# hyx1999/SAM-Decoding

Measured on AMD Instinct MI355X. Metric: tokens/sec (+ mean accepted tokens), Vicuna-7B bs=1, samd_sam_only draft+verify, higher is better.
Workload: dtype f16

## Files before the change

include/samd_hip.h:

```cpp
#ifndef SAMD_HIP_H
#define SAMD_HIP_H

#include <stdint.h>

#ifdef __cplusplus
extern "C" {
#endif

#define SAMD_OK 0
#define SAMD_E_INVALID (-1)
#define SAMD_E_CAPACITY (-2)
#define SAMD_E_HIP (-3)
#define SAMD_E_IO (-4)
#define SAMD_E_NODEVICE (-5)

#define SAMD_MAX_DRAFT 128
#define SAMD_TOPK 8

#define SAMD_REP_DMETA 0
#define SAMD_REP_VERDICT 16
#define SAMD_REP_TOKENS 24
#define SAMD_REP_KVINDEX 152
#define SAMD_REP_COUNTERS 280
#define SAMD_REP_META 288
// ... 77 lines not shown
    uint64_t mask_hi[SAMD_MAX_DRAFT];
    int32_t retrieve[SAMD_MAX_DRAFT * SAMD_MAX_DRAFT];
} samd_draft_host_t;

typedef struct samd_verdict_host {
    int32_t best, accept, next_node, next_token;
    int32_t tokens[SAMD_MAX_DRAFT];
    int32_t kv_index[SAMD_MAX_DRAFT];
} samd_verdict_host_t;

int samd_session_create(int32_t max_tokens, samd_session_t **out);
void samd_session_free(samd_session_t *s);
int samd_session_reset(samd_session_t *s, void *stream);

int samd_dyn_add_tokens(samd_session_t *s, const int32_t *d_tokens, int32_t n, const int32_t *d_n, void *stream);
int samd_dyn_walk(samd_session_t *s, const int32_t *d_tokens, int32_t n, int32_t commit, int32_t *d_out, void *stream);
int samd_session_static_walk(samd_session_t *s, const samd_static_t *sam, const int32_t *d_tokens, int32_t n,
                             const int32_t *d_n, int32_t commit, int32_t *d_out, void *stream);
int samd_session_export(samd_session_t *s, int64_t out_info[10], int32_t *h_link, int32_t *h_length, int32_t *h_minend,
                        int32_t *h_deg, int32_t *h_edge_tok, int32_t *h_edge_dst, int32_t *h_text, void *stream);
int samd_session_set_cursors(samd_session_t *s, int32_t dyn_index, int32_t dyn_length, int32_t st_index,
                             int32_t st_length, void *stream);

int samd_session_set_start_token(samd_session_t *s, const int32_t *d_src, void *stream);

int samd_session_draft(samd_session_t *s, const samd_static_t *sam, const samd_params_t *p,
                       const int32_t *d_start_token, void *stream);
int samd_session_draft_seq(samd_session_t *s, const samd_params_t *p, int32_t index, int32_t match, int32_t start_token,
                           void *stream);
int samd_session_draft_tree(samd_session_t *s, const samd_static_t *sam, const samd_params_t *p, int32_t index,
                            int32_t match, int32_t start_token, void *stream);
int samd_session_draft_fixed(samd_session_t *s, const samd_static_t *sam, const samd_params_t *p, int32_t source,
                             int32_t index, int32_t start_token, void *stream);
int samd_session_set_draft(samd_session_t *s, const int32_t *d_tokens, const int32_t *d_parent, int32_t n, int32_t type,
                           void *stream);
int samd_session_read_draft(samd_session_t *s, samd_draft_host_t *out, void *stream);
int samd_session_set_draft_if_deferred(samd_session_t *s, const int32_t *d_tokens, const int32_t *d_parent, int32_t n,
                                       int32_t reverse_leaves, void *stream);
int samd_tree_attention_signal(const void *d_q, const void *d_k_cache, const void *d_v_cache, void *d_out, int32_t dtype, int32_t n_q_pad,
                               int32_t n_heads, int32_t n_kv_heads, int32_t head_dim, int64_t max_len, const uint64_t *d_mask,
                               const int32_t *d_cache_length, const int32_t *d_n, float scale, void *d_workspace, int64_t workspace_bytes,
                               int32_t *d_arrive, void *stream);
int samd_gemm_cs_residual_early(const void *d_A, const void *d_Wg, int32_t N, int32_t K, void *d_x, float *d_ssq, int32_t dtype, const int32_t *d_counter,
                                int32_t *d_epoch, int32_t arrivals, void *stream);

int samd_session_report_target(samd_session_t *s, int32_t **out_host);
int samd_report_wait(const int32_t *h_report, int32_t last_seq, int64_t timeout_us);

int samd_session_report_async(samd_session_t *s, int32_t *h_dst, void *stream);

int samd_session_device_views(samd_session_t *s, void *out[16]);

int samd_tree_buffers(const int32_t *d_parent, int32_t n, int32_t reverse_leaves, int32_t *d_position, uint64_t *d_mask,
                      uint8_t *d_mask_bool, int32_t *d_retrieve, int32_t *d_shape, void *stream);


int samd_argmax_rows(const void *d_logits, int32_t dtype, int32_t rows, int64_t vocab, int64_t row_stride,
                     const int32_t *d_rows, int32_t *d_out, void *stream);

int samd_session_accept(samd_session_t *s, const int32_t *d_node_argmax, void *stream);
int samd_session_candidates(samd_session_t *s, int64_t *d_candidates, int32_t *d_rowmap, int32_t capacity, void *stream);
int samd_session_step_given(samd_session_t *s, const samd_static_t *sam, const samd_params_t *p, const int32_t *d_best_accept,
                            const int32_t *d_next_token, void *stream);
int samd_session_read_verdict(samd_session_t *s, samd_verdict_host_t *out, void *stream);
int samd_session_commit(samd_session_t *s, const samd_static_t *sam, void *stream);
int samd_session_step(samd_session_t *s, const samd_static_t *sam, const samd_params_t *p,
// ... 188 lines not shown
```

sam-decoding_amd/csrc/sam_device.h:

```cpp
#pragma once
#include <hip/hip_runtime.h>
#include "samd_common.h"

#define WAVE 64
#define PATH_PAD 255

__device__ __forceinline__ int lane_id() { return threadIdx.x & (WAVE - 1); }

__device__ __forceinline__ void wave_mem_sync() { __builtin_amdgcn_fence(__ATOMIC_SEQ_CST, "workgroup"); }

__device__ __forceinline__ int spill_search(const SamEdge *tab, int deg, int tok) {
    const uint32_t m = samd_spill_slots(deg);
    uint32_t h = samd_spill_hash(tok, m);
    for (uint32_t probes = 0; probes < m; probes++) {
        const SamEdge e = tab[h];
        if (e.tok == tok) return e.dst;
        if (e.tok == -1) return -1;
        h = (h + 1) & (m - 1);
    }
    return -1;
}

__device__ __forceinline__ int st_transfer(const StaticDev &S, int &idx, int &len, int tok) {
    int visited = 0;
// ... 561 lines not shown
    double h_prob[8 * SAMD_MAX_DRAFT + 8];
    int h_tok[8 * SAMD_MAX_DRAFT + 8], h_idx[8 * SAMD_MAX_DRAFT + 8], h_anc[8 * SAMD_MAX_DRAFT + 8], h_dep[8 * SAMD_MAX_DRAFT + 8];
    int dep_cnt[SAMD_MAX_DRAFT + 2];
    int c_tok[SAMD_TOPK], c_dst[SAMD_TOPK], c_cnt[SAMD_TOPK];
    int pop_ok, pop_tok, pop_idx, pop_anc, pop_dep; double pop_prob;
};

__device__ __forceinline__ void path_fill(StepShared &sh, int rows) {
    const uint4 pad = make_uint4(0xFFFFFFFFu, 0xFFFFFFFFu, 0xFFFFFFFFu, 0xFFFFFFFFu);
    static_assert(PATH_PAD == 255 && SAMD_MAX_DRAFT % 16 == 0, "");
    uint4 *p = reinterpret_cast<uint4 *>(&sh.path[0][0]);
    for (int k = lane_id(); k < rows * (SAMD_MAX_DRAFT / 16); k += WAVE) p[k] = pad;
}

__device__ __forceinline__ int seq_draft_var(StepShared &sh, const int *text, int n_text, int endpos, int n, int start) {
    const int lo = endpos + 1;
    int hi = endpos + n; hi = hi > n_text ? n_text : hi;
    const int m = 1 + (hi > lo ? hi - lo : 0);
    for (int i = lane_id(); i < m; i += WAVE) { sh.tokens[i] = (i == 0) ? start : text[endpos + i]; sh.parent[i] = i - 1; }
    __syncthreads();
    return m;
}

__device__ __forceinline__ int seq_draft_fixed(StepShared &sh, const int *text, int n_text, int endpos, int n_predicts, int start) {
    for (int i = lane_id(); i < n_predicts; i += WAVE) {
        int v = 0;
        if (i == 0) v = start; else if (endpos + i < n_text) v = text[endpos + i];
        sh.tokens[i] = v; sh.parent[i] = i - 1;
    }
    __syncthreads();
    return n_predicts;
}

__device__ __forceinline__ void hq_set(StepShared &sh, int pos, double p, int t, int i, int a, int d) {
    sh.h_prob[pos] = p; sh.h_tok[pos] = t; sh.h_idx[pos] = i; sh.h_anc[pos] = a; sh.h_dep[pos] = d;
}
__device__ __forceinline__ void hq_move(StepShared &sh, int dst, int src) {
    sh.h_prob[dst] = sh.h_prob[src]; sh.h_tok[dst] = sh.h_tok[src]; sh.h_idx[dst] = sh.h_idx[src];
    sh.h_anc[dst] = sh.h_anc[src]; sh.h_dep[dst] = sh.h_dep[src];
}
__device__ __forceinline__ void hq_siftdown(StepShared &sh, int start, int pos, double p, int t, int i, int a, int d) {
    while (pos > start) {
        const int par = (pos - 1) >> 1;
        if (p < sh.h_prob[par]) { hq_move(sh, pos, par); pos = par; continue; }
        break;
    }
    hq_set(sh, pos, p, t, i, a, d);
}
__device__ __forceinline__ void hq_push(StepShared &sh, int &hn, double p, int t, int i, int a, int d) {
    hn++;
    hq_siftdown(sh, 0, hn - 1, p, t, i, a, d);
}
__device__ __forceinline__ void hq_pop(StepShared &sh, int &hn, double &p, int &t, int &i, int &a, int &d) {
    hn--;
    const double lp = sh.h_prob[hn]; const int lt = sh.h_tok[hn], li = sh.h_idx[hn], la = sh.h_anc[hn], ld = sh.h_dep[hn];
    if (hn == 0) { p = lp; t = lt; i = li; a = la; d = ld; return; }
    p = sh.h_prob[0]; t = sh.h_tok[0]; i = sh.h_idx[0]; a = sh.h_anc[0]; d = sh.h_dep[0];
    int pos = 0, child = 1;
    while (child < hn) {
        const int right = child + 1;
        if (right < hn && !(sh.h_prob[child] < sh.h_prob[right])) child = right;
        hq_move(sh, pos, child); pos = child; child = 2 * pos + 1;
    }
    hq_siftdown(sh, 0, pos, lp, lt, li, la, ld);
}

__device__ __forceinline__ int tree_draft(StepShared &sh, const StaticDev &S, int index, int n, int K, int start) {
    const int lane = lane_id();
    int hn = 0, m = 0;
    for (int k = lane; k < SAMD_MAX_DRAFT + 2; k += WAVE) sh.dep_cnt[k] = 0;
    __syncthreads();
    if (lane == 0) hq_push(sh, hn, -1.0, start, index, -1, 0);
    __syncthreads();
    while (m != n) {
        if (lane == 0) {
            int ok = 0; double p = 0; int t = 0, i = 0, a = 0, d = 0;
            while (hn > 0) {
                hq_pop(sh, hn, p, t, i, a, d);
                if (sh.dep_cnt[d] + 1 > K) continue;
                sh.dep_cnt[d] += 1; ok = 1; break;
            }
            sh.pop_ok = ok; sh.pop_prob = p; sh.pop_tok = t; sh.pop_idx = i; sh.pop_anc = a; sh.pop_dep = d;
        }
        __syncthreads();
        if (!sh.pop_ok) break;
        const int cur = m;
        if (lane == 0) { sh.tokens[m] = sh.pop_tok; sh.parent[m] = sh.pop_anc; }
        m++;
        if (m == n) break;
        const int4 *np = reinterpret_cast<const int4 *>(S.nodes + sh.pop_idx);
        const int4 w1 = np[1];
        const int le = lane < SAMD_INLINE_EDGES ? lane : 0;
        const int2 ie = *reinterpret_cast<const int2 *>(reinterpret_cast<const int *>(np) + SAMD_EDGE_WORD(le));
        const int sp = reinterpret_cast<const int *>(np)[14];
        const int cnt_pre = S.topk_cnt ? S.topk_cnt[(size_t)sh.pop_idx * SAMD_TOPK + (lane & (SAMD_TOPK - 1))] : 0;
        int kk = w1.y < SAMD_TOPK ? w1.y : SAMD_TOPK; kk = kk < K ? kk : K;
        if (lane < kk) {
            int tk = ie.x, ds = ie.y;
            if (lane >= SAMD_INLINE_EDGES) { const SamEdge ed = S.spill[sp + lane - SAMD_INLINE_EDGES]; tk = ed.tok; ds = ed.dst; }
            sh.c_tok[lane] = tk; sh.c_dst[lane] = ds; sh.c_cnt[lane] = S.topk_cnt ? cnt_pre : S.nodes[ds].aux;
        }
        __syncthreads();
        if (lane == 0) {
            const double cnt_sum = (double)w1.x, pp = sh.pop_prob;
            const int dep = sh.pop_dep + 1;
            for (int j = 0; j < kk; j++) {
                const double n_prob = (double)sh.c_cnt[j] / cnt_sum;
                hq_push(sh, hn, pp * n_prob, sh.c_tok[j], sh.c_dst[j], cur, dep);
            }
        }
        __syncthreads();
    }
    __syncthreads();
    return m;
}

__device__ __forceinline__ void build_buffers(StepShared &sh, int n, int reverse, int &n_leaves, int &max_depth) {
    const int lane = lane_id();
    if (lane == 0) { sh.child_mask[0] = 0ull; sh.child_mask[1] = 0ull; }
    __syncthreads();
    for (int i = lane; i < n; i += WAVE) {
        const int p = sh.parent[i];
        if (i == 0) sh.parent[0] = -1;
        else if (p < 0 || p >= i) sh.parent[i] = 0;
    }
    __syncthreads();
    int md = 0;
    for (int i = lane; i < n; i += WAVE) {
        int depth = 0; unsigned long long m = 0ull, mh = 0ull;
        for (int j = i; j != -1; j = sh.parent[j]) { if (j < 64) m |= 1ull << j; else mh |= 1ull << (j - 64); depth++; }
        depth -= 1;
        sh.position[i] = depth; sh.mask[i] = m; sh.mask_hi[i] = mh;
        if (i > 0) { const int p = sh.parent[i]; atomicOr(&sh.child_mask[p >> 6], 1ull << (p & 63)); }
        md = depth + 1 > md ? depth + 1 : md;
    }
    for (int o = 32; o > 0; o >>= 1) { int v = __shfl_xor(md, o); md = v > md ? v : md; }
    __syncthreads();
    const int n0 = n < 64 ? n : 64, n1 = n > 64 ? n - 64 : 0;
    const unsigned long long valid0 = n0 >= 64 ? ~0ull : ((1ull << n0) - 1ull), valid1 = n1 >= 64 ? ~0ull : ((1ull << n1) - 1ull);
    const unsigned long long leaf0 = valid0 & ~sh.child_mask[0], leaf1 = valid1 & ~sh.child_mask[1];
    const int nl0 = __popcll(leaf0), nl = nl0 + __popcll(leaf1);
    path_fill(sh, nl);
    __syncthreads();
    for (int i = lane; i < n; i += WAVE) {
        const bool is_leaf = i < 64 ? ((leaf0 >> i) & 1ull) : ((leaf1 >> (i - 64)) & 1ull);
        if (!is_leaf) continue;
        int r = i < 64 ? __popcll(leaf0 & ((1ull << i) - 1ull)) : nl0 + __popcll(leaf1 & ((1ull << (i - 64)) - 1ull));
        if (reverse) r = nl - 1 - r;
        for (int j = i; j != -1; j = sh.parent[j]) sh.path[r][sh.position[j]] = (unsigned char)j;
    }
    __syncthreads();
    n_leaves = nl; max_depth = md;
}

__device__ __forceinline__ void store_draft(const SessionDev &D, StepShared &sh, int type, int n, int n_leaves, int max_depth,
                                            int idx_dyn, int m_dyn, int idx_st, int m_st, int reverse) {
    const int i = lane_id();
    for (int k = i; k < SAMD_MAX_DRAFT; k += WAVE) {
        if (k < n) { D.tokens[k] = sh.tokens[k]; D.parent[k] = sh.parent[k]; D.position[k] = sh.position[k]; D.mask[k] = sh.mask[k]; D.mask_hi[k] = sh.mask_hi[k]; }
        else { D.tokens[k] = 0; D.parent[k] = k - 1; D.position[k] = 0; D.mask[k] = 0ull; D.mask_hi[k] = 0ull; }
    }
    for (int k = i; k < n_leaves * max_depth; k += WAVE) {
        const unsigned char v = sh.path[k / max_depth][k % max_depth];
        D.retrieve[k] = v == PATH_PAD ? -1 : (int)v;
    }
    if (i == 0) {
        D.dmeta[D_TYPE] = type; D.dmeta[D_N] = n; D.dmeta[D_NLEAVES] = n_leaves; D.dmeta[D_MAXDEPTH] = max_depth;
        D.dmeta[D_IDX_DYN] = idx_dyn; D.dmeta[D_MATCH_DYN] = m_dyn; D.dmeta[D_IDX_ST] = idx_st; D.dmeta[D_MATCH_ST] = m_st;
        D.dmeta[8] = reverse;
    }
}

__device__ __forceinline__ void do_draft(const SessionDev &D, const StaticDev &S, bool have_static, const samd_params_t &P,
                                         StepShared &sh, int start) {
    int id = D.meta[M_CUR_IDX], md = D.meta[M_CUR_LEN];
    dyn_transfer(D, id, md, start);
    int is = 0, ms = 0;
    if (have_static) { is = D.meta[M_ST_IDX]; ms = D.meta[M_ST_LEN]; st_transfer(S, is, ms, start); }
    ms -= P.len_bias;
    int type, n;
    if (P.variant == 0) {
        if (md >= ms || !have_static) {
            type = 0;
            n = seq_draft_var(sh, D.text, D.meta[M_NTEXT], D.minend[id], draft_size(md, P.alpha, P.max_predicts), start);
        } else {
            type = 1;
            n = tree_draft(sh, S, is, draft_size(ms, P.alpha, P.max_predicts), P.K, start);
        }
    } else {
        const int best = md > ms ? md : ms;
        if (best >= P.len_threshold) {
            type = 0;
            if (md >= ms || !have_static) {
                int a = id;
                if (a != 0) {
                    const int maxlen = D.meta[M_MAXLEN];
                    int to_end = maxlen - D.minend[a];
                    while (D.link[a] != 0 && P.n_predicts > to_end) { a = D.link[a]; to_end = maxlen - D.minend[a]; }
                }
                n = seq_draft_fixed(sh, D.text, D.meta[M_NTEXT], D.minend[a], P.n_predicts, start);
            } else {
                n = seq_draft_fixed(sh, S.text, S.n_text, S.nodes[is].aux, P.n_predicts, start);
            }
        } else {
            type = 2; n = 1;
            if (lane_id() == 0) { sh.tokens[0] = start; sh.parent[0] = -1; }
            __syncthreads();
        }
    }
    int nl, mxd;
    build_buffers(sh, n, 0, nl, mxd);
    store_draft(D, sh, type, n, nl, mxd, id, md, is, ms, 0);
}

__device__ __forceinline__ void do_accept(const SessionDev &D, StepShared &sh, const int *node_argmax, int type, int n,
                                          int n_leaves, int max_depth, int &accept_out, int &next_token_out) {
    const int i = lane_id();
    for (int k = i; k < n; k += WAVE) sh.node_argmax[k] = node_argmax[k];
    __syncthreads();
    int key = -1;
    for (int row = i; row < n_leaves; row += WAVE) {
        int acc = 0;
        for (int j = 1; j < max_depth; j++) {
            const int cj = sh.path[row][j], pj = sh.path[row][j - 1];
            const int cand = cj == PATH_PAD ? 0 : sh.tokens[cj];
            const int am = sh.node_argmax[pj == PATH_PAD ? n - 1 : pj];
            if (cand != am) break;
            acc++;
        }
        const int kk = acc * SAMD_MAX_DRAFT + (SAMD_MAX_DRAFT - 1 - row);
        key = kk > key ? kk : key;
    }
    for (int o = 32; o > 0; o >>= 1) { int v = __shfl_xor(key, o); key = v > key ? v : key; }
    const int best_acc = key / SAMD_MAX_DRAFT, best = SAMD_MAX_DRAFT - 1 - (key % SAMD_MAX_DRAFT);
    const int a = best_acc + 1;
    for (int k = i; k < a; k += WAVE) {
        const int node = sh.path[best][k];
        const int tk = node == PATH_PAD ? 0 : sh.tokens[node];
        sh.accepted[k] = tk;
        D.acc_tokens[k] = tk;
        D.kv_index[k] = node == PATH_PAD ? -1 : node;
    }
    const int nn_raw = sh.path[best][best_acc];
    const int nn = nn_raw == PATH_PAD ? n - 1 : nn_raw;
    const int next_token = sh.node_argmax[nn];
// ... 42 lines not shown
```

sam-decoding_amd/csrc/sam_kernels.hip:

```cpp
#include <hip/hip_runtime.h>
#include <cstdio>
#include <cstdlib>
#include <cstring>
#include <ctime>
#include <functional>
#include <vector>
#include <hipcub/hipcub.hpp>
#include "sam_device.h"

#define HIPCHK(x) do { hipError_t e_ = (x); if (e_ != hipSuccess) { samd_set_error("%s: %s", #x, hipGetErrorString(e_)); return SAMD_E_HIP; } } while (0)
#define LAUNCHCHK() do { hipError_t e_ = hipGetLastError(); if (e_ != hipSuccess) { samd_set_error("kernel launch: %s", hipGetErrorString(e_)); return SAMD_E_HIP; } } while (0)

static inline StaticDev static_view(const samd_static_t *s) {
    StaticDev v;
    if (!s) { memset(&v, 0, sizeof(v)); return v; }
    v.nodes = s->d_nodes; v.root_next = s->d_root; v.spill = s->d_spill; v.text = s->d_text;
    v.n_states = (int32_t)s->n_states; v.vocab = (int32_t)s->vocab; v.n_text = (int32_t)s->n_text; v.kind = s->kind;
    v.chain = (const uint4 *)s->d_chain; v.chain_w = samd_chain_w(s->vocab);
    v.root16 = (const uint4 *)s->d_root16; v.bigram = (const uint4 *)s->d_d1hash; v.bigram_mask = s->n_d1hash > 0 ? (uint32_t)(s->n_d1hash - 1) : 0u;
    v.rc_bits = (const uint32_t *)s->d_rc_bits;
    v.ehash = (const uint4 *)s->d_ehash; v.edge_mask = s->n_ehash > 0 ? (uint32_t)(s->n_ehash - 1) : 0u;
    v.topk_cnt = (const int32_t *)s->d_topk_cnt;
    v.hot = s->d_d1hash ? (const uint4 *)s->d_hot : nullptr; v.blocks = s->d_d1hash ? (const uint4 *)s->d_blocks : nullptr; v.eb_tok_bits = samd_eb_tok_bits(s->vocab);
    return v;
// ... 49 lines not shown
            const int4 w0 = reinterpret_cast<const int4 *>(nodes + s + j)[0];
            if (w0.z >= 0 && (unsigned)w0.z < LOW && (long long)w0.w == s + j + 1) {
                const bool flagged = (w0.y & SAMD_SINGLE) && w0.x > 0 && nodes[w0.x].link == 0;
                tokw[j] = (unsigned)w0.z | (flagged ? 0u : HI);
            } else alive = false;
        } else alive = false;
    }
    uint4 o;
    if constexpr (W == 8) { o.x = tokw[0] | (tokw[1] << 16); o.y = tokw[2] | (tokw[3] << 16); o.z = tokw[4] | (tokw[5] << 16); o.w = tokw[6] | (tokw[7] << 16); }
    else { o.x = tokw[0]; o.y = tokw[1]; o.z = tokw[2]; o.w = tokw[3]; }
    chain[s] = o;
}

enum { OP_RESET = 1, OP_ADD = 2, OP_DYN_WALK = 4, OP_ST_WALK = 8, OP_DRAFT = 16, OP_ACCEPT = 32, OP_COMMIT = 64,
       OP_DRAFT_SEQ = 128, OP_DRAFT_TREE = 256, OP_DRAFT_FIXED = 512, OP_SET_DRAFT = 1024, OP_SET_CURSORS = 2048,
       OP_BUFFERS_ONLY = 4096, OP_ACCEPT_GIVEN = 8192 };

struct StepArgs {
    int ops;
    const int32_t *tokens;
    const int32_t *parents;
    const int32_t *d_n;
    int n;
    int commit;
    int32_t *out2;
    const int32_t *start_token;
    const int32_t *node_argmax;
    const int32_t *given;
    const int32_t *given_next;
    int index, match, start, source, type, reverse;
    int c0, c1, c2, c3;
    int have_static;
    int only_if_deferred;
    int push_report;
};

__device__ __forceinline__ void load_draft(const SessionDev &D, StepShared &sh, int &type, int &n, int &nl, int &md) {
    const int i = lane_id();
    type = D.dmeta[D_TYPE]; n = D.dmeta[D_N]; nl = D.dmeta[D_NLEAVES]; md = D.dmeta[D_MAXDEPTH];
    for (int k = i; k < n; k += WAVE) { sh.tokens[k] = D.tokens[k]; sh.parent[k] = D.parent[k]; }
    path_fill(sh, nl < SAMD_MAX_DRAFT ? (nl < 1 ? 1 : nl) : SAMD_MAX_DRAFT);
    __syncthreads();
    for (int k = i; k < nl * md; k += WAVE) {
        const int v = D.retrieve[k];
        sh.path[k / md][k % md] = v < 0 ? PATH_PAD : (unsigned char)v;
    }
    __syncthreads();
}

__global__ __launch_bounds__(64) void k_session(SessionDev D, StaticDev S, samd_params_t P, StepArgs A) {
    __shared__ StepShared sh;
    const int lane = lane_id();

    if (A.ops & OP_RESET) {
        for (uint32_t k = lane; k <= D.hmask; k += WAVE) D.hkey[k] = SAMD_HEMPTY;
        if (lane == 0) {
            D.link[0] = -1; D.length[0] = 0; D.minend[0] = 0; D.head[0] = -1; D.tail[0] = -1;
            D.text[0] = -1;
            for (int k = 0; k < M_COUNT; k++) D.meta[k] = 0;
            D.meta[M_NSTATES] = 1; D.meta[M_NTEXT] = 1;
            for (int k = 0; k < D_COUNT; k++) D.dmeta[k] = 0;
            for (int k = 0; k < V_COUNT; k++) D.verdict[k] = 0;
            for (int k = 0; k < C_COUNT; k++) D.counters[k] = 0;
            D.start_token[0] = 0; D.cache_length[0] = 0;
        }
        wave_mem_sync();
    }
    if (A.ops & OP_SET_CURSORS) {
        if (lane == 0) { D.meta[M_CUR_IDX] = A.c0; D.meta[M_CUR_LEN] = A.c1; D.meta[M_ST_IDX] = A.c2; D.meta[M_ST_LEN] = A.c3; }
        wave_mem_sync();
    }
    int n_in = A.d_n ? A.d_n[0] : A.n;
    unsigned long long t_prev = __builtin_amdgcn_s_memrealtime();
    auto phase_done = [&](int slot) {
        const unsigned long long t = __builtin_amdgcn_s_memrealtime();
        if (lane == 0) D.counters[slot] += (int)(t - t_prev);
        t_prev = t;
    };

    if (A.ops & OP_ACCEPT) {
        int type, n, nl, md, a, nt;
        load_draft(D, sh, type, n, nl, md);
        do_accept(D, sh, A.node_argmax, type, n, nl, md, a, nt);
        wave_mem_sync();
// ... 8 lines not shown
    }
    if (A.ops & OP_COMMIT) {
        const int a = D.verdict[V_ACCEPT];
        for (int k = lane; k < a; k += WAVE) sh.accepted[k] = D.acc_tokens[k];
        __syncthreads();
        dyn_add_tokens(D, sh.accepted, a);
        wave_mem_sync();
        phase_done(C_T_DYN);
        if (A.have_static) {
            int is = D.meta[M_ST_IDX], ms = D.meta[M_ST_LEN];
            st_transfer_tokens(S, is, ms, sh.accepted, a);
            if (lane == 0) { D.meta[M_ST_IDX] = is; D.meta[M_ST_LEN] = ms; }
        }
        wave_mem_sync();
        phase_done(C_T_STATIC);
    }
    if (A.ops & OP_ADD) dyn_add_tokens(D, A.tokens, n_in);
    if (A.ops & OP_DYN_WALK) {
        int ci = D.meta[M_CUR_IDX], cl = D.meta[M_CUR_LEN];
        for (int i = 0; i < n_in; i++) dyn_transfer(D, ci, cl, A.tokens[i]);
        if (A.commit && lane == 0) { D.meta[M_CUR_IDX] = ci; D.meta[M_CUR_LEN] = cl; }
        if (A.out2 && lane == 0) { A.out2[0] = ci; A.out2[1] = cl; }
        wave_mem_sync();
    }
    if (A.ops & OP_ST_WALK) {
        int is = D.meta[M_ST_IDX], ms = D.meta[M_ST_LEN];
        if (A.have_static) st_transfer_tokens(S, is, ms, A.tokens, n_in);
        else if (n_in > 0) { is = 0; ms = 0; }
        if (A.commit && lane == 0) { D.meta[M_ST_IDX] = is; D.meta[M_ST_LEN] = ms; }
        if (A.out2 && lane == 0) { A.out2[0] = is; A.out2[1] = ms; }
        wave_mem_sync();
    }
    if (A.ops & OP_DRAFT) {
        do_draft(D, S, A.have_static != 0, P, sh, A.start_token[0]);
        wave_mem_sync();
        phase_done(C_T_DRAFT);
    }
    if (A.ops & OP_DRAFT_SEQ) {
        const int n = seq_draft_var(sh, D.text, D.meta[M_NTEXT], D.minend[A.index], draft_size(A.match, P.alpha, P.max_predicts), A.start);
        int nl, mxd; build_buffers(sh, n, 0, nl, mxd);
        store_draft(D, sh, 0, n, nl, mxd, A.index, A.match, 0, 0, 0);
    }
    if (A.ops & OP_DRAFT_TREE) {
        const int n = tree_draft(sh, S, A.index, draft_size(A.match, P.alpha, P.max_predicts), P.K, A.start);
        int nl, mxd; build_buffers(sh, n, 0, nl, mxd);
        store_draft(D, sh, 1, n, nl, mxd, 0, 0, A.index, A.match, 0);
    }
    if (A.ops & OP_DRAFT_FIXED) {
        int n;
        if (A.source == 0) {
            int a = A.index;
            if (a != 0) {
                const int maxlen = D.meta[M_MAXLEN];
                int to_end = maxlen - D.minend[a];
                while (D.link[a] != 0 && P.n_predicts > to_end) { a = D.link[a]; to_end = maxlen - D.minend[a]; }
            }
            n = seq_draft_fixed(sh, D.text, D.meta[M_NTEXT], D.minend[a], P.n_predicts, A.start);
            if (lane == 0) D.dmeta[9] = a;
        } else {
            n = seq_draft_fixed(sh, S.text, S.n_text, S.nodes[A.index].aux, P.n_predicts, A.start);
        }
        int nl, mxd; build_buffers(sh, n, 0, nl, mxd);
        store_draft(D, sh, 0, n, nl, mxd, A.index, 0, A.index, 0, 0);
    }
    if ((A.ops & OP_SET_DRAFT) && !(A.only_if_deferred && D.dmeta[D_TYPE] != 2)) {
        for (int k = lane; k < A.n; k += WAVE) { sh.tokens[k] = A.tokens[k]; sh.parent[k] = A.parents[k]; }
        __syncthreads();
        int nl, mxd; build_buffers(sh, A.n, A.reverse, nl, mxd);
        store_draft(D, sh, A.type, A.n, nl, mxd, 0, 0, 0, 0, A.reverse);
    }
    if (A.push_report && D.h_report) {
        wave_mem_sync();
        for (int k = lane; k < SAMD_REPORT_INTS; k += WAVE)
            __hip_atomic_store(D.h_report + k, D.dmeta[k], __ATOMIC_RELAXED, __HIP_MEMORY_SCOPE_SYSTEM);
        __builtin_amdgcn_fence(__ATOMIC_RELEASE, "");
        asm volatile("s_waitcnt vmcnt(0)" ::: "memory");
        if (lane == 0) {
            const int seq = D.push_seq[0] + 1;
            D.push_seq[0] = seq;
// ... 637 lines not shown
    if (s->h_report_host) (void)hipHostFree(s->h_report_host);
    free(s);
}

int samd_session_report_target(samd_session_t *s, int32_t **out_host) {
    if (!s || !out_host) return SAMD_E_INVALID;
    if (!s->h_report_host) {
        void *h = nullptr, *d = nullptr;
        const size_t bytes = 4 * (SAMD_REPORT_INTS + 16);
        if (hipHostMalloc(&h, bytes, hipHostMallocCoherent | hipHostMallocMapped) != hipSuccess) { samd_set_error("hipHostMalloc(report target) failed"); return SAMD_E_HIP; }
        memset(h, 0, bytes);
        if (hipHostGetDevicePointer(&d, h, 0) != hipSuccess) { (void)hipHostFree(h); samd_set_error("hipHostGetDevicePointer(report target) failed"); return SAMD_E_HIP; }
        s->h_report_host = (int32_t *)h;
        s->dev.h_report = (int32_t *)d;
    }
    *out_host = s->h_report_host;
    return SAMD_OK;
}

int samd_report_wait(const int32_t *h_report, int32_t last_seq, int64_t timeout_us) {
    if (!h_report) return SAMD_E_INVALID;
    const volatile int32_t *seq = h_report + SAMD_REPORT_INTS;
    timespec t0; clock_gettime(CLOCK_MONOTONIC, &t0);
    for (unsigned spin = 0;; spin++) {
        if (*seq != last_seq) { __atomic_thread_fence(__ATOMIC_ACQUIRE); return SAMD_OK; }
        __builtin_ia32_pause();
        if ((spin & 1023u) == 1023u) {
            timespec t; clock_gettime(CLOCK_MONOTONIC, &t);
            if ((t.tv_sec - t0.tv_sec) * 1000000ll + (t.tv_nsec - t0.tv_nsec) / 1000 > timeout_us) return SAMD_E_CAPACITY;
        }
    }
}

static int launch_session(samd_session_t *s, const samd_static_t *sam, const samd_params_t *p, StepArgs &A, void *stream) {
    if (!s) { samd_set_error("null session"); return SAMD_E_INVALID; }
    if (sam && !sam->uploaded) { samd_set_error("static automaton not uploaded"); return SAMD_E_INVALID; }
    samd_params_t P; memset(&P, 0, sizeof(P));
    if (p) P = *p;
    if (p && (P.max_predicts > SAMD_MAX_DRAFT || P.n_predicts > SAMD_MAX_DRAFT || P.max_predicts < 0 || P.n_predicts < 0)) {
        samd_set_error("max_predicts / n_predicts must be in [0, %d]", SAMD_MAX_DRAFT); return SAMD_E_INVALID;
    }
    A.have_static = sam ? 1 : 0;
    hipLaunchKernelGGL(k_session, dim3(1), dim3(WAVE), 0, (hipStream_t)stream, s->dev, static_view(sam), P, A);
    LAUNCHCHK();
    return SAMD_OK;
}

int samd_session_reset(samd_session_t *s, void *stream) {
    StepArgs A; memset(&A, 0, sizeof(A)); A.ops = OP_RESET;
    return launch_session(s, nullptr, nullptr, A, stream);
}

int samd_dyn_add_tokens(samd_session_t *s, const int32_t *d_tokens, int32_t n, const int32_t *d_n, void *stream) {
    if (n < 0 || (!d_tokens && n > 0)) return SAMD_E_INVALID;
    StepArgs A; memset(&A, 0, sizeof(A)); A.ops = OP_ADD; A.tokens = d_tokens; A.n = n; A.d_n = d_n;
    return launch_session(s, nullptr, nullptr, A, stream);
}

int samd_dyn_walk(samd_session_t *s, const int32_t *d_tokens, int32_t n, int32_t commit, int32_t *d_out, void *stream) {
    if (n < 0 || (!d_tokens && n > 0)) return SAMD_E_INVALID;
    StepArgs A; memset(&A, 0, sizeof(A)); A.ops = OP_DYN_WALK; A.tokens = d_tokens; A.n = n; A.commit = commit; A.out2 = d_out;
    return launch_session(s, nullptr, nullptr, A, stream);
}

int samd_session_static_walk(samd_session_t *s, const samd_static_t *sam, const int32_t *d_tokens, int32_t n,
                             const int32_t *d_n, int32_t commit, int32_t *d_out, void *stream) {
    if (n < 0 || (!d_tokens && n > 0)) return SAMD_E_INVALID;
    StepArgs A; memset(&A, 0, sizeof(A)); A.ops = OP_ST_WALK; A.tokens = d_tokens; A.n = n; A.d_n = d_n; A.commit = commit; A.out2 = d_out;
    return launch_session(s, sam, nullptr, A, stream);
}

int samd_session_set_cursors(samd_session_t *s, int32_t di, int32_t dl, int32_t si, int32_t sl, void *stream) {
    StepArgs A; memset(&A, 0, sizeof(A)); A.ops = OP_SET_CURSORS; A.c0 = di; A.c1 = dl; A.c2 = si; A.c3 = sl;
    return launch_session(s, nullptr, nullptr, A, stream);
}
// ... 210 lines not shown
```

sam-decoding_amd/csrc/samd_common.h:

```cpp
#pragma once
#include <stdint.h>
#include <stddef.h>
#include "../../include/samd_hip.h"

#define SAMD_ABI_VERSION 2
#define SAMD_INLINE_EDGES 5
#define SAMD_SPILL_HEAD 3

#define SAMD_SINGLE 0x40000000
#define SAMD_RUN 0x20000000
#define SAMD_LEN_MASK 0x1FFFFFFF
struct __attribute__((aligned(64))) SamNode {
    int32_t link, length, e0_tok, e0_dst;
    int32_t aux, deg, e1_tok, e1_dst;
    int32_t e2_tok, e2_dst, e3_tok, e3_dst;
    int32_t e4_tok, e4_dst, spill, reserved;
};
static_assert(sizeof(SamNode) == 64, "SamNode must be one 64-byte line");
#define SAMD_EDGE_WORD(k) ((k) == 0 ? 2 : 4 + 2 * (k))

struct SamEdge { int32_t tok, dst; };

#if defined(__HIPCC__)
#define SAMD_HD __host__ __device__
// ... 25 lines not shown
#define SAMD_EB_KIND_SHIFT 28
#define SAMD_EB_ROOTCHILD 0x40000000u
#define SAMD_EB_DISPLACED 0x80000000u
#define SAMD_BG_DISPLACED 0x20000000u
SAMD_HD static inline uint32_t samd_eb_base(uint32_t ref) { return (ref & SAMD_EB_IDX_MASK) << 2; }
SAMD_HD static inline uint32_t samd_eb_mask(uint32_t ref) { return (1u << (ref >> 27)) - 1u; }
SAMD_HD static inline uint32_t samd_eb_hash(int32_t tok) { uint32_t h = (uint32_t)tok * 0x9E3779B1u; return h ^ (h >> 15); }
SAMD_HD static inline int samd_eb_tok_bits(int64_t vocab) { int b = 8; while (b < 31 && ((int64_t)1 << b) - 1 < vocab) b++; return b; }

struct StaticDev {
    const SamNode *nodes;
    const int32_t *root_next;
    const SamEdge *spill;
    const int32_t *text;
    int32_t n_states, vocab, n_text, kind;
    const uint4 *chain;
    int32_t chain_w;
    const uint4 *root16;
    const uint4 *bigram;
    uint32_t bigram_mask;
    const uint32_t *rc_bits;
    const uint4 *ehash;
    uint32_t edge_mask;
    const uint4 *hot;
    const uint4 *blocks;
    int32_t eb_tok_bits;
    const int32_t *topk_cnt;
};

enum {
    M_NSTATES = 0, M_NEDGES, M_NTEXT, M_LAST, M_MAXLEN, M_CUR_IDX, M_CUR_LEN, M_ST_IDX, M_ST_LEN, M_ERROR,
    M_COUNT = 16
};
enum { D_TYPE = 0, D_N, D_NLEAVES, D_MAXDEPTH, D_IDX_DYN, D_MATCH_DYN, D_IDX_ST, D_MATCH_ST, D_COUNT = 16 };
enum { V_BEST = 0, V_ACCEPT, V_NEXT_NODE, V_NEXT_TOKEN, V_KV_START, V_IS_TREE, V_COUNT = 8 };
enum { C_STEPS = 0, C_TOKENS, C_SEQ_STEPS, C_TREE_STEPS, C_T_ACCEPT, C_T_DYN, C_T_STATIC, C_T_DRAFT, C_COUNT = 8 };

#define SAMD_HEMPTY 0xFFFFFFFFFFFFFFFFull

struct SessionDev {
    int32_t *link, *length, *minend, *head, *tail;
    uint64_t *hkey;
    int32_t *hdst, *hnext;
    int32_t *text;
    int32_t *meta;
    int32_t *tokens, *parent, *position;
    uint64_t *mask;
    uint64_t *mask_hi;
    int32_t *retrieve;
    int32_t *dmeta;
    int32_t *verdict;
    int32_t *acc_tokens, *kv_index;
    int32_t *start_token, *cache_length;
    int32_t *counters;
    uint32_t hmask;
    int32_t cap_states, cap_text, max_tokens;
    int32_t *h_report;
    int32_t *push_seq;
};

struct samd_session {
    SessionDev dev;
    void *arena;
    size_t arena_bytes;
    int32_t max_tokens;
    int32_t *h_report_host;
};
// ... 73 lines not shown
```

sam-decoding_amd/samd_hip/__init__.py:

```python
import ctypes as C
import os

import numpy as np

_HERE = os.path.dirname(os.path.abspath(__file__))
LIB_PATH = os.environ.get("SAMD_HIP_LIB") or os.path.join(_HERE, "libsamd_hip.so")
MAX_DRAFT = 128
TILE_ROWS = 64
TOPK = 8
REP_DMETA, REP_VERDICT, REP_TOKENS, REP_KVINDEX, REP_COUNTERS, REP_META, REPORT_INTS = 0, 16, 24, 152, 280, 288, 304
KIND_COUNT, KIND_ENDPOS = 0, 1
F16, BF16, F32 = 0, 1, 2

_lib = None


class SamdError(RuntimeError):
    pass


class Params(C.Structure):
    _fields_ = [("variant", C.c_int32), ("max_predicts", C.c_int32), ("alpha", C.c_double), ("K", C.c_int32),
                ("len_bias", C.c_int32), ("n_predicts", C.c_int32), ("len_threshold", C.c_int32),
                ("static_null", C.c_int32), ("reserved", C.c_int32)]
# ... 37 lines not shown
    "samd_static_from_tables": (C.c_int, [_I32, _I64, _VP, _VP, _VP, _VP, _VP, _VP, _VP, _I64, _VP]),
    "samd_static_save": (C.c_int, [_VP, C.c_char_p]),
    "samd_static_load": (C.c_int, [C.c_char_p, _VP]),
    "samd_static_free": (None, [_VP]),
    "samd_static_upload": (C.c_int, [_VP]),
    "samd_static_info": (C.c_int, [_VP, _VP]),
    "samd_static_from_pickle": (C.c_int, [C.c_char_p, _I32, _VP, _VP]),
    "samd_static_derived_info": (C.c_int, [_VP, _VP]),
    "samd_static_edge_blocks_info": (C.c_int, [_VP, _VP]),
    "samd_static_set_bigram_slots": (C.c_int, [_VP, _I32, _VP]),
    "samd_static_export": (C.c_int, [_VP, _VP, _VP, _VP, _VP, _VP, _VP]),
    "samd_static_device_image": (C.c_int, [_VP, _VP, _VP]),
    "samd_static_alloc_like": (C.c_int, [_VP, _VP]),
    "samd_static_host_image": (C.c_int, [_VP, _VP, _VP]),
    "samd_static_from_host_image": (C.c_int, [_VP, _VP, _VP]),
    "samd_static_adopt_device": (C.c_int, [_VP, _VP, _VP]),
    "samd_static_walk": (C.c_int, [_VP, _VP, _VP, _I32, _I32, _I32, _VP, _VP]),
    "samd_static_walk_counted": (C.c_int, [_VP, _VP, _VP, _I32, _I32, _I32, _VP, _VP]),
    "samd_static_lookup_batch": (C.c_int, [_VP, _VP, _VP, _I32, _I32, _VP, _VP, _VP]),
    "samd_static_walk_streams": (C.c_int, [_VP, _VP, _VP, _I32, _I32, _I32, _VP, _VP]),
    "samd_static_walk_streams_counted": (C.c_int, [_VP, _VP, _VP, _I32, _I32, _I32, _VP, _VP]),
    "samd_session_create": (C.c_int, [_I32, _VP]),
    "samd_session_free": (None, [_VP]),
    "samd_session_reset": (C.c_int, [_VP, _VP]),
    "samd_dyn_add_tokens": (C.c_int, [_VP, _VP, _I32, _VP, _VP]),
    "samd_dyn_walk": (C.c_int, [_VP, _VP, _I32, _I32, _VP, _VP]),
    "samd_session_static_walk": (C.c_int, [_VP, _VP, _VP, _I32, _VP, _I32, _VP, _VP]),
    "samd_session_export": (C.c_int, [_VP, _VP, _VP, _VP, _VP, _VP, _VP, _VP, _VP, _VP]),
    "samd_session_set_cursors": (C.c_int, [_VP, _I32, _I32, _I32, _I32, _VP]),
    "samd_session_draft": (C.c_int, [_VP, _VP, _VP, _VP, _VP]),
    "samd_session_draft_seq": (C.c_int, [_VP, _VP, _I32, _I32, _I32, _VP]),
    "samd_session_draft_tree": (C.c_int, [_VP, _VP, _VP, _I32, _I32, _I32, _VP]),
    "samd_session_draft_fixed": (C.c_int, [_VP, _VP, _VP, _I32, _I32, _I32, _VP]),
    "samd_session_set_draft": (C.c_int, [_VP, _VP, _VP, _I32, _I32, _VP]),
    "samd_session_read_draft": (C.c_int, [_VP, _VP, _VP]),
    "samd_session_set_draft_if_deferred": (C.c_int, [_VP, _VP, _VP, _I32, _I32, _VP]),
    "samd_session_report_async": (C.c_int, [_VP, _VP, _VP]),
    "samd_session_set_start_token": (C.c_int, [_VP, _VP, _VP]),
    "samd_scripted_argmax": (C.c_int, [_VP, _VP, _I32, _I32, _VP, _VP]),
    "samd_embed_rows_ssq": (C.c_int, [_VP, _VP, _VP, _VP, _I32, _I32, _I32, _I32, _VP]),
    "samd_embed_rows_ssq_rope": (C.c_int, [_VP, _VP, _VP, _VP, _I32, _I32, _I32, _I32, _VP, _VP, _VP, _VP, _VP, _I32, _I32, _I32, _VP]),
    "samd_gemm_qkv_rope_norm": (C.c_int, [_VP, _VP, _VP, C.c_float, _VP, _I32, _I32, _VP, _VP, _VP, _VP, _VP, _VP, _I32, _I32, _I32, _I64, _I32, _VP]),
    "samd_gemm_qkv_rope_norm_vt": (C.c_int, [_VP, _VP, _VP, C.c_float, _VP, _I32, _I32, _VP, _VP, _VP, _VP, _VP, _VP, _I32, _I32, _I32, _I64, _I32, _VP]),
    "samd_gemm_pairs_silu_norm": (C.c_int, [_VP, _VP, _VP, C.c_float, _VP, _I32, _I32, _I32, _VP, _I32, _VP]),
    "samd_gemm_cs_residual": (C.c_int, [_VP, _VP, _I32, _I32, _I32, _VP, _VP, _I32, _VP]),
    "samd_gemm_cs_residual_early": (C.c_int, [_VP, _VP, _I32, _I32, _VP, _VP, _I32, _VP, _VP, _I32, _VP]),
    "samd_tree_attention_signal": (C.c_int, [_VP, _VP, _VP, _VP, _I32, _I32, _I32, _I32, _I32, _I64, _VP, _VP, _VP, _F32, _VP, _I64, _VP, _VP]),
    "samd_session_report_target": (C.c_int, [_VP, C.POINTER(_VP)]),
    "samd_report_wait": (C.c_int, [_VP, _I32, _I64]),
    "samd_scripted_logits": (C.c_int, [_VP, _VP, _VP, _I32, _I32, _I64, _I32, _VP]),
    "samd_scripted_logits_order1": (C.c_int, [_VP, _VP, _VP, _I32, _I32, _I64, _I32, _VP]),
    "samd_session_device_views": (C.c_int, [_VP, _VP]),
    "samd_tree_buffers": (C.c_int, [_VP, _I32, _I32, _VP, _VP, _VP, _VP, _VP, _VP]),
    "samd_argmax_rows": (C.c_int, [_VP, _I32, _I32, _I64, _I64, _VP, _VP, _VP]),
    "samd_session_accept": (C.c_int, [_VP, _VP, _VP]),
    "samd_session_read_verdict": (C.c_int, [_VP, _VP, _VP]),
    "samd_session_commit": (C.c_int, [_VP, _VP, _VP]),
    "samd_session_step": (C.c_int, [_VP, _VP, _VP, _VP, _VP]),
    "samd_session_step_given": (C.c_int, [_VP, _VP, _VP, _VP, _VP, _VP]),
    "samd_session_candidates": (C.c_int, [_VP, _VP, _VP, _I32, _VP]),
    "samd_session_set_cache_length": (C.c_int, [_VP, _I32, _VP]),
    "samd_session_get_cache_length": (C.c_int, [_VP, _VP, _VP]),
    "samd_kv_compact": (C.c_int, [_VP, _VP, _I32, _I32, _I64, _I32, _I32, _VP]),
    "samd_kv_compact_indices": (C.c_int, [_VP, _I32, _I32, _I64, _I32, _I32, _I32, _VP, _I32, _VP]),
    "samd_tree_attention_workspace": (_I64, [_I32, _I32, _I32]),
    "samd_tree_attention": (C.c_int, [_VP, _VP, _VP, _VP, _I32, _I32, _I32, _I32, _I32, _I64, _VP, _VP, _VP, _F32,
# ... 70 lines not shown
                            "(hipcc --offload-arch=gfx950); there is no CPU fallback")
        L = C.CDLL(LIB_PATH)
        for name, (res, args) in _PROTOS.items():
            fn = getattr(L, name)
            fn.restype = res
            fn.argtypes = args
        _lib = L
    return _lib


def check(rc):
    if rc != 0:
        msg = lib().samd_last_error()
        raise SamdError(f"libsamd_hip error {rc}: {msg.decode() if msg else ''}")


def host_waits_by_spinning(device_index=None):
    if os.environ.get("SAMD_SPIN_WAIT", "1") == "0":
        return False
    import logging
    log = logging.getLogger("samd_hip")
    try:
        import torch
        rc = lib().samd_host_wait_spin(-1 if device_index is None else int(device_index))
    except (ImportError, OSError, AttributeError, SamdError) as e:
        log.warning("host_waits_by_spinning: not applied (%s)", e)
        return False
    if rc != 0:
        msg = lib().samd_last_error()
        log.warning("host_waits_by_spinning: not applied (rc %d: %s)", rc, msg.decode() if msg else "")
    return rc == 0


def require_gpu():
    if lib().samd_device_count() < 1:
        raise SamdError("no MI355X / HIP device visible: the SAM-Decoding hot path has no CPU fallback")


def _np_i32(a):
    return np.ascontiguousarray(a, dtype=np.int32)


def _ptr(a):
    if a is None:
        return None
    if isinstance(a, C.c_void_p):
        return a
    if isinstance(a, np.ndarray):
        return a.ctypes.data_as(C.c_void_p)
    if hasattr(a, "data_ptr"):
        return C.c_void_p(a.data_ptr())
    return C.c_void_p(int(a))


def current_stream():
    import torch
    return C.c_void_p(torch.cuda.current_stream().cuda_stream)


def torch_dtype_code(dtype):
    import torch
    return {torch.float16: F16, torch.bfloat16: BF16, torch.float32: F32}[dtype]


class StaticAutomaton:

# ... 317 lines not shown
```

Measured before the change: 814.0.

## Prefetch child SAM node records into LDS during tree draft expansion

During the best-first tree draft, the kernel now issues asynchronous global-to-LDS loads for each pushed child's node record and top-k counts into a ring of LDS slots. When a child is later popped, its data is read from LDS after waiting on only as many outstanding loads as needed, rather than paying a dependent global load per pop. This is meant to hide the per-step latency of walking the static automaton. In exchange it adds LDS usage, inline assembly with manual vmcnt bookkeeping, and replaces block barriers with wave-level barriers, which is delicate for correctness.

```diff
diff --git a/include/samd_hip.h b/include/samd_hip.h
--- a/include/samd_hip.h
+++ b/include/samd_hip.h
@@ -133,6 +133,7 @@
                             int32_t match, int32_t start_token, void *stream);
 int samd_session_draft_fixed(samd_session_t *s, const samd_static_t *sam, const samd_params_t *p, int32_t source,
                              int32_t index, int32_t start_token, void *stream);
+int samd_debug_set_tree_record_ring(int depth);
 int samd_session_set_draft(samd_session_t *s, const int32_t *d_tokens, const int32_t *d_parent, int32_t n, int32_t type,
                            void *stream);
 int samd_session_read_draft(samd_session_t *s, samd_draft_host_t *out, void *stream);
diff --git a/sam-decoding_amd/csrc/sam_device.h b/sam-decoding_amd/csrc/sam_device.h
--- a/sam-decoding_amd/csrc/sam_device.h
+++ b/sam-decoding_amd/csrc/sam_device.h
@@ -617,85 +617,160 @@
     return n_predicts;
 }
 
-__device__ __forceinline__ void hq_set(StepShared &sh, int pos, double p, int t, int i, int a, int d) {
-    sh.h_prob[pos] = p; sh.h_tok[pos] = t; sh.h_idx[pos] = i; sh.h_anc[pos] = a; sh.h_dep[pos] = d;
-}
-__device__ __forceinline__ void hq_move(StepShared &sh, int dst, int src) {
+#define SAMD_TREE_RING 16
+#define TREE_NO_RECORD 0xFFFF
+struct TreeRecords {
+    __attribute__((aligned(16))) unsigned char rec[SAMD_TREE_RING][SAMD_TOPK][128];
+    int slot_seq[SAMD_TREE_RING];
+    unsigned short h_rec[8 * SAMD_MAX_DRAFT + 8];
+    int pop_rec, pop_lag;
+};
+static_assert(sizeof(StepShared) + sizeof(TreeRecords) <= 65536, "k_session's static LDS must stay within 64 KB");
+static_assert(8 * (SAMD_MAX_DRAFT + 1) + 7 <= 0xFFFF, "record ids must fit TreeRecords::h_rec");
+
+__device__ __forceinline__ void wave_lds_sync() {
+    asm volatile("s_waitcnt lgkmcnt(0)" ::: "memory");
+    __builtin_amdgcn_s_barrier();
+    asm volatile("" ::: "memory");
+}
+
+#define TREE_LANDED(x) asm volatile("" : "+v"(x))
+
+__device__ __forceinline__ bool tree_request_records(TreeRecords &tr, const StaticDev &S, int slot, int ds, bool on) {
+    const int q = lane_id() & 7;
+    if (__ballot(on && (ds < 0 || ds >= S.n_states)) != 0ull) return false;
+    if (on) {
+        const char *src = q < 4 ? reinterpret_cast<const char *>(S.nodes + ds) + 16 * q
+                                : reinterpret_cast<const char *>(S.topk_cnt + (size_t)ds * SAMD_TOPK) + 16 * (q - 4);
+        typedef __attribute__((address_space(3))) void *lptr_t;
+        const unsigned base = __builtin_amdgcn_readfirstlane((unsigned)(uintptr_t)(lptr_t)&tr.rec[slot][0][0]);
+        unsigned keep;
+        asm volatile("s_mov_b32 %0, m0\n\ts_mov_b32 m0, %2\n\ts_nop 0\n\tglobal_load_lds_dwordx4 %1, off\n\ts_mov_b32 m0, %0"
+                     : "=&s"(keep) : "v"(src), "s"(base) : "memory");
+    }
+    return true;
+}
+
+__device__ __forceinline__ void hq_set(StepShared &sh, unsigned short *hr, int pos, double p, int t, int i, int a, int d, int r) {
+    sh.h_prob[pos] = p; sh.h_tok[pos] = t; sh.h_idx[pos] = i; sh.h_anc[pos] = a; sh.h_dep[pos] = d; hr[pos] = (unsigned short)r;
+}
+__device__ __forceinline__ void hq_move(StepShared &sh, unsigned short *hr, int dst, int src) {
     sh.h_prob[dst] = sh.h_prob[src]; sh.h_tok[dst] = sh.h_tok[src]; sh.h_idx[dst] = sh.h_idx[src];
-    sh.h_anc[dst] = sh.h_anc[src]; sh.h_dep[dst] = sh.h_dep[src];
-}
-__device__ __forceinline__ void hq_siftdown(StepShared &sh, int start, int pos, double p, int t, int i, int a, int d) {
+    sh.h_anc[dst] = sh.h_anc[src]; sh.h_dep[dst] = sh.h_dep[src]; hr[dst] = hr[src];
+}
+__device__ __forceinline__ void hq_siftdown(StepShared &sh, unsigned short *hr, int start, int pos, double p, int t, int i, int a, int d, int r) {
     while (pos > start) {
         const int par = (pos - 1) >> 1;
-        if (p < sh.h_prob[par]) { hq_move(sh, pos, par); pos = par; continue; }
+        if (p < sh.h_prob[par]) { hq_move(sh, hr, pos, par); pos = par; continue; }
         break;
     }
-    hq_set(sh, pos, p, t, i, a, d);
-}
-__device__ __forceinline__ void hq_push(StepShared &sh, int &hn, double p, int t, int i, int a, int d) {
+    hq_set(sh, hr, pos, p, t, i, a, d, r);
+}
+__device__ __forceinline__ void hq_push(StepShared &sh, unsigned short *hr, int &hn, double p, int t, int i, int a, int d, int r) {
     hn++;
-    hq_siftdown(sh, 0, hn - 1, p, t, i, a, d);
-}
-__device__ __forceinline__ void hq_pop(StepShared &sh, int &hn, double &p, int &t, int &i, int &a, int &d) {
+    hq_siftdown(sh, hr, 0, hn - 1, p, t, i, a, d, r);
+}
+__device__ __forceinline__ void hq_pop(StepShared &sh, unsigned short *hr, int &hn, double &p, int &t, int &i, int &a, int &d, int &r) {
     hn--;
-    const double lp = sh.h_prob[hn]; const int lt = sh.h_tok[hn], li = sh.h_idx[hn], la = sh.h_anc[hn], ld = sh.h_dep[hn];
-    if (hn == 0) { p = lp; t = lt; i = li; a = la; d = ld; return; }
-    p = sh.h_prob[0]; t = sh.h_tok[0]; i = sh.h_idx[0]; a = sh.h_anc[0]; d = sh.h_dep[0];
+    const double lp = sh.h_prob[hn]; const int lt = sh.h_tok[hn], li = sh.h_idx[hn], la = sh.h_anc[hn], ld = sh.h_dep[hn], lr = hr[hn];
+    if (hn == 0) { p = lp; t = lt; i = li; a = la; d = ld; r = lr; return; }
+    p = sh.h_prob[0]; t = sh.h_tok[0]; i = sh.h_idx[0]; a = sh.h_anc[0]; d = sh.h_dep[0]; r = hr[0];
     int pos = 0, child = 1;
     while (child < hn) {
         const int right = child + 1;
         if (right < hn && !(sh.h_prob[child] < sh.h_prob[right])) child = right;
-        hq_move(sh, pos, child); pos = child; child = 2 * pos + 1;
-    }
-    hq_siftdown(sh, 0, pos, lp, lt, li, la, ld);
-}
-
-__device__ __forceinline__ int tree_draft(StepShared &sh, const StaticDev &S, int index, int n, int K, int start) {
+        hq_move(sh, hr, pos, child); pos = child; child = 2 * pos + 1;
+    }
+    hq_siftdown(sh, hr, 0, pos, lp, lt, li, la, ld, lr);
+}
+
+__device__ __forceinline__ int tree_draft(StepShared &sh, TreeRecords &tr, int ring, const StaticDev &S, int index, int n, int K, int start,
+                                          int &from_records) {
     const int lane = lane_id();
     int hn = 0, m = 0;
+    from_records = 0;
+    if (!S.topk_cnt) ring = 0;
+    const int rmask = ring - 1;
+    int seq = 0;
+    if (lane < SAMD_TREE_RING) tr.slot_seq[lane] = -1;
+    asm volatile("s_waitcnt vmcnt(0)" ::: "memory");
+    if (ring && n > 1 && tree_request_records(tr, S, 0, index, lane < 6)) {
+        if (lane == 0) tr.slot_seq[0] = 0;
+        seq = 1;
+    }
     for (int k = lane; k < SAMD_MAX_DRAFT + 2; k += WAVE) sh.dep_cnt[k] = 0;
-    __syncthreads();
-    if (lane == 0) hq_push(sh, hn, -1.0, start, index, -1, 0);
-    __syncthreads();
+    wave_lds_sync();
+    if (lane == 0) hq_push(sh, tr.h_rec, hn, -1.0, start, index, -1, 0, seq ? 0 : TREE_NO_RECORD);
+    wave_lds_sync();
     while (m != n) {
         if (lane == 0) {
-            int ok = 0; double p = 0; int t = 0, i = 0, a = 0, d = 0;
+            int ok = 0; double p = 0; int t = 0, i = 0, a = 0, d = 0, r = 0;
             while (hn > 0) {
-                hq_pop(sh, hn, p, t, i, a, d);
+                hq_pop(sh, tr.h_rec, hn, p, t, i, a, d, r);
                 if (sh.dep_cnt[d] + 1 > K) continue;
                 sh.dep_cnt[d] += 1; ok = 1; break;
             }
             sh.pop_ok = ok; sh.pop_prob = p; sh.pop_tok = t; sh.pop_idx = i; sh.pop_anc = a; sh.pop_dep = d;
-        }
-        __syncthreads();
+            const int rs = r >> 3;
+            const bool live = ring && tr.slot_seq[rs & rmask] == rs;
+            tr.pop_rec = live ? (((rs & rmask) << 3) + (r & 7)) * 128 : -1;
+            tr.pop_lag = seq - 1 - rs;
+        }
+        wave_lds_sync();
         if (!sh.pop_ok) break;
         const int cur = m;
         if (lane == 0) { sh.tokens[m] = sh.pop_tok; sh.parent[m] = sh.pop_anc; }
         m++;
         if (m == n) break;
-        const int4 *np = reinterpret_cast<const int4 *>(S.nodes + sh.pop_idx);
-        const int4 w1 = np[1];
         const int le = lane < SAMD_INLINE_EDGES ? lane : 0;
-        const int2 ie = *reinterpret_cast<const int2 *>(reinterpret_cast<const int *>(np) + SAMD_EDGE_WORD(le));
-        const int sp = reinterpret_cast<const int *>(np)[14];
-        const int cnt_pre = S.topk_cnt ? S.topk_cnt[(size_t)sh.pop_idx * SAMD_TOPK + (lane & (SAMD_TOPK - 1))] : 0;
-        int kk = w1.y < SAMD_TOPK ? w1.y : SAMD_TOPK; kk = kk < K ? kk : K;
+        const int pr = __builtin_amdgcn_readfirstlane(tr.pop_rec);
+        int aux, deg, sp, cnt_pre; int2 ie;
+        if (pr >= 0) {
+            from_records++;
+            const int lag = __builtin_amdgcn_readfirstlane(tr.pop_lag);
+            if (lag <= 0) asm volatile("s_waitcnt vmcnt(0)" ::: "memory");
+            else if (lag == 1) asm volatile("s_waitcnt vmcnt(1)" ::: "memory");
+            else if (lag == 2) asm volatile("s_waitcnt vmcnt(2)" ::: "memory");
+            else asm volatile("s_waitcnt vmcnt(3)" ::: "memory");
+            const int *rw = reinterpret_cast<const int *>(&tr.rec[0][0][0] + pr);
+            aux = rw[4]; deg = rw[5]; sp = rw[14];
+            ie = *reinterpret_cast<const int2 *>(rw + SAMD_EDGE_WORD(le));
+            cnt_pre = rw[16 + (lane & (SAMD_TOPK - 1))];
+        } else {
+            const int4 *np = reinterpret_cast<const int4 *>(S.nodes + sh.pop_idx);
+            const int4 w1 = np[1];
+            aux = w1.x; deg = w1.y;
+            ie = *reinterpret_cast<const int2 *>(reinterpret_cast<const int *>(np) + SAMD_EDGE_WORD(le));
+            sp = reinterpret_cast<const int *>(np)[14];
+            cnt_pre = S.topk_cnt ? S.topk_cnt[(size_t)sh.pop_idx * SAMD_TOPK + (lane & (SAMD_TOPK - 1))] : 0;
+            TREE_LANDED(aux); TREE_LANDED(deg); TREE_LANDED(ie.x); TREE_LANDED(ie.y); TREE_LANDED(sp); TREE_LANDED(cnt_pre);
+        }
+        int kk = deg < SAMD_TOPK ? deg : SAMD_TOPK; kk = kk < K ? kk : K;
         if (lane < kk) {
-            int tk = ie.x, ds = ie.y;
-            if (lane >= SAMD_INLINE_EDGES) { const SamEdge ed = S.spill[sp + lane - SAMD_INLINE_EDGES]; tk = ed.tok; ds = ed.dst; }
-            sh.c_tok[lane] = tk; sh.c_dst[lane] = ds; sh.c_cnt[lane] = S.topk_cnt ? cnt_pre : S.nodes[ds].aux;
-        }
-        __syncthreads();
+            int tk = ie.x, ds = ie.y, cn = cnt_pre;
+            if (lane >= SAMD_INLINE_EDGES) { const SamEdge ed = S.spill[sp + lane - SAMD_INLINE_EDGES]; tk = ed.tok; ds = ed.dst; TREE_LANDED(tk); TREE_LANDED(ds); }
+            if (!S.topk_cnt) { cn = S.nodes[ds].aux; TREE_LANDED(cn); }
+            sh.c_tok[lane] = tk; sh.c_dst[lane] = ds; sh.c_cnt[lane] = cn;
+        }
+        wave_lds_sync();
+        bool request = ring && kk > 0 && m < n - 1;
+        if (request) {
+            const int j = lane >> 3;
+            request = tree_request_records(tr, S, seq & rmask, j < kk ? sh.c_dst[j] : 0, j < kk && (lane & 7) < 6);
+            if (lane == 0) tr.slot_seq[seq & rmask] = request ? seq : -1;
+        }
         if (lane == 0) {
-            const double cnt_sum = (double)w1.x, pp = sh.pop_prob;
+            const double cnt_sum = (double)aux, pp = sh.pop_prob;
             const int dep = sh.pop_dep + 1;
             for (int j = 0; j < kk; j++) {
                 const double n_prob = (double)sh.c_cnt[j] / cnt_sum;
-                hq_push(sh, hn, pp * n_prob, sh.c_tok[j], sh.c_dst[j], cur, dep);
-            }
-        }
-        __syncthreads();
-    }
+                hq_push(sh, tr.h_rec, hn, pp * n_prob, sh.c_tok[j], sh.c_dst[j], cur, dep, request ? seq * 8 + j : TREE_NO_RECORD);
+            }
+        }
+        if (request) seq++;
+        wave_lds_sync();
+    }
+    asm volatile("s_waitcnt vmcnt(0)" ::: "memory");
     __syncthreads();
     return m;
 }
@@ -757,20 +832,20 @@
 }
 
 __device__ __forceinline__ void do_draft(const SessionDev &D, const StaticDev &S, bool have_static, const samd_params_t &P,
-                                         StepShared &sh, int start) {
+                                         StepShared &sh, TreeRecords &tr, int ring, int start) {
     int id = D.meta[M_CUR_IDX], md = D.meta[M_CUR_LEN];
     dyn_transfer(D, id, md, start);
     int is = 0, ms = 0;
     if (have_static) { is = D.meta[M_ST_IDX]; ms = D.meta[M_ST_LEN]; st_transfer(S, is, ms, start); }
     ms -= P.len_bias;
-    int type, n;
+    int type, n, from_records = 0;
     if (P.variant == 0) {
         if (md >= ms || !have_static) {
             type = 0;
             n = seq_draft_var(sh, D.text, D.meta[M_NTEXT], D.minend[id], draft_size(md, P.alpha, P.max_predicts), start);
         } else {
             type = 1;
-            n = tree_draft(sh, S, is, draft_size(ms, P.alpha, P.max_predicts), P.K, start);
+            n = tree_draft(sh, tr, ring, S, is, draft_size(ms, P.alpha, P.max_predicts), P.K, start, from_records);
         }
     } else {
         const int best = md > ms ? md : ms;
@@ -796,6 +871,7 @@
     int nl, mxd;
     build_buffers(sh, n, 0, nl, mxd);
     store_draft(D, sh, type, n, nl, mxd, id, md, is, ms, 0);
+    if (lane_id() == 0) D.dmeta[D_TREE_RECORDS] = from_records;
 }
 
 __device__ __forceinline__ void do_accept(const SessionDev &D, StepShared &sh, const int *node_argmax, int type, int n,
diff --git a/sam-decoding_amd/csrc/sam_kernels.hip b/sam-decoding_amd/csrc/sam_kernels.hip
--- a/sam-decoding_amd/csrc/sam_kernels.hip
+++ b/sam-decoding_amd/csrc/sam_kernels.hip
@@ -105,6 +105,7 @@
     int c0, c1, c2, c3;
     int have_static;
     int only_if_deferred;
+    int tree_ring;
     int push_report;
 };
 
@@ -123,6 +124,7 @@
 
 __global__ __launch_bounds__(64) void k_session(SessionDev D, StaticDev S, samd_params_t P, StepArgs A) {
     __shared__ StepShared sh;
+    __shared__ TreeRecords tr;
     const int lane = lane_id();
 
     if (A.ops & OP_RESET) {
@@ -197,7 +199,7 @@
         wave_mem_sync();
     }
     if (A.ops & OP_DRAFT) {
-        do_draft(D, S, A.have_static != 0, P, sh, A.start_token[0]);
+        do_draft(D, S, A.have_static != 0, P, sh, tr, A.tree_ring, A.start_token[0]);
         wave_mem_sync();
         phase_done(C_T_DRAFT);
     }
@@ -207,9 +209,11 @@
         store_draft(D, sh, 0, n, nl, mxd, A.index, A.match, 0, 0, 0);
     }
     if (A.ops & OP_DRAFT_TREE) {
-        const int n = tree_draft(sh, S, A.index, draft_size(A.match, P.alpha, P.max_predicts), P.K, A.start);
+        int from_records;
+        const int n = tree_draft(sh, tr, A.tree_ring, S, A.index, draft_size(A.match, P.alpha, P.max_predicts), P.K, A.start, from_records);
         int nl, mxd; build_buffers(sh, n, 0, nl, mxd);
         store_draft(D, sh, 1, n, nl, mxd, 0, 0, A.index, A.match, 0);
+        if (lane == 0) D.dmeta[D_TREE_RECORDS] = from_records;
     }
     if (A.ops & OP_DRAFT_FIXED) {
         int n;
@@ -913,6 +917,16 @@
     }
 }
 
+static int g_tree_ring = SAMD_TREE_RING;
+
+int samd_debug_set_tree_record_ring(int depth) {
+    if (depth < 0 || depth > SAMD_TREE_RING || (depth & (depth - 1)) != 0) {
+        samd_set_error("tree record ring depth must be 0 or a power of two <= %d", SAMD_TREE_RING); return SAMD_E_INVALID;
+    }
+    __atomic_store_n(&g_tree_ring, depth, __ATOMIC_RELAXED);
+    return SAMD_OK;
+}
+
 static int launch_session(samd_session_t *s, const samd_static_t *sam, const samd_params_t *p, StepArgs &A, void *stream) {
     if (!s) { samd_set_error("null session"); return SAMD_E_INVALID; }
     if (sam && !sam->uploaded) { samd_set_error("static automaton not uploaded"); return SAMD_E_INVALID; }
@@ -922,6 +936,7 @@
         samd_set_error("max_predicts / n_predicts must be in [0, %d]", SAMD_MAX_DRAFT); return SAMD_E_INVALID;
     }
     A.have_static = sam ? 1 : 0;
+    A.tree_ring = __atomic_load_n(&g_tree_ring, __ATOMIC_RELAXED);
     hipLaunchKernelGGL(k_session, dim3(1), dim3(WAVE), 0, (hipStream_t)stream, s->dev, static_view(sam), P, A);
     LAUNCHCHK();
     return SAMD_OK;
diff --git a/sam-decoding_amd/csrc/samd_common.h b/sam-decoding_amd/csrc/samd_common.h
--- a/sam-decoding_amd/csrc/samd_common.h
+++ b/sam-decoding_amd/csrc/samd_common.h
@@ -81,7 +81,7 @@
     M_NSTATES = 0, M_NEDGES, M_NTEXT, M_LAST, M_MAXLEN, M_CUR_IDX, M_CUR_LEN, M_ST_IDX, M_ST_LEN, M_ERROR,
     M_COUNT = 16
 };
-enum { D_TYPE = 0, D_N, D_NLEAVES, D_MAXDEPTH, D_IDX_DYN, D_MATCH_DYN, D_IDX_ST, D_MATCH_ST, D_COUNT = 16 };
+enum { D_TYPE = 0, D_N, D_NLEAVES, D_MAXDEPTH, D_IDX_DYN, D_MATCH_DYN, D_IDX_ST, D_MATCH_ST, D_TREE_RECORDS = 10, D_COUNT = 16 };
 enum { V_BEST = 0, V_ACCEPT, V_NEXT_NODE, V_NEXT_TOKEN, V_KV_START, V_IS_TREE, V_COUNT = 8 };
 enum { C_STEPS = 0, C_TOKENS, C_SEQ_STEPS, C_TREE_STEPS, C_T_ACCEPT, C_T_DYN, C_T_STATIC, C_T_DRAFT, C_COUNT = 8 };
 
diff --git a/sam-decoding_amd/samd_hip/__init__.py b/sam-decoding_amd/samd_hip/__init__.py
--- a/sam-decoding_amd/samd_hip/__init__.py
+++ b/sam-decoding_amd/samd_hip/__init__.py
@@ -93,6 +93,7 @@
     "samd_session_draft_seq": (C.c_int, [_VP, _VP, _I32, _I32, _I32, _VP]),
     "samd_session_draft_tree": (C.c_int, [_VP, _VP, _VP, _I32, _I32, _I32, _VP]),
     "samd_session_draft_fixed": (C.c_int, [_VP, _VP, _VP, _I32, _I32, _I32, _VP]),
+    "samd_debug_set_tree_record_ring": (C.c_int, [C.c_int]),
     "samd_session_set_draft": (C.c_int, [_VP, _VP, _VP, _I32, _I32, _VP]),
     "samd_session_read_draft": (C.c_int, [_VP, _VP, _VP]),
     "samd_session_set_draft_if_deferred": (C.c_int, [_VP, _VP, _VP, _I32, _I32, _VP]),
@@ -229,6 +230,14 @@
     return rc == 0
 
 
+TREE_RECORD_RING = 16
+D_TREE_RECORDS = 10
+
+
+def debug_set_tree_record_ring(depth=TREE_RECORD_RING):
+    check(lib().samd_debug_set_tree_record_ring(int(depth)))
+
+
 def require_gpu():
     if lib().samd_device_count() < 1:
         raise SamdError("no MI355X / HIP device visible: the SAM-Decoding hot path has no CPU fallback")
```

After: 813.9. About the same (-0.0%).
